# pierotofy/OpenSplat

Hardware: NVIDIA H100
Metric: fwd_bwd_mpixel_per_s (higher is better)
Workload: dtype f32

## Files before the change

opensplat_b200/csrc/raster_bwd.cu:

```cuda
#include "raster_common.cuh"

int gsb_blend_grid(const void *kernel, int num_tiles);

namespace {

__device__ __forceinline__ float rcp_approx(float x) {
    float y;
    asm("rcp.approx.ftz.f32 %0, %1;" : "=f"(y) : "f"(x));
    return y;
}

__device__ __forceinline__ void zero_row(float *grad_rows, int k) {
    float4 *row = reinterpret_cast<float4 *>(grad_rows + (size_t)k * GSB_GRAD_ROW_FLOATS);
    const float4 z = make_float4(0.f, 0.f, 0.f, 0.f);
    row[0] = z; row[1] = z; row[2] = z;
}

constexpr int BWD_MIN_BLOCKS = 6;
template <bool SAT>
__global__ void __launch_bounds__(RK_THREADS, BWD_MIN_BLOCKS)
rasterize_backward_kernel(int img_h, int img_w, int tiles_x, int num_tiles,
                          const int2 *__restrict__ tile_bins, const GsbRecord *__restrict__ records,
                          const float *__restrict__ background, const float *__restrict__ final_Ts,
                          const int *__restrict__ final_idx, const float *__restrict__ v_output,
                          const float *__restrict__ v_output_alpha, float *__restrict__ grad_rows,
                          unsigned *__restrict__ tile_counter, const int *__restrict__ tile_order) {
    __shared__ WarpRing rings[RK_WARPS];
    const int warp = threadIdx.x >> 5, lane = threadIdx.x & 31;
    WarpRing &ring = rings[warp];
    if (lane == 0) {
#pragma unroll
        for (int s = 0; s < RK_STAGES; ++s) mbar_init(&ring.full[s], 1);
        mbar_fence_init();
    }
    __syncwarp();
    const float bg0 = __ldg(background), bg1 = __ldg(background + 1), bg2 = __ldg(background + 2);
    unsigned gchunk = 0;

    while (true) {
        int tile = 0;
        if (lane == 0) tile = (int)atomicAdd(tile_counter, 1u);
        tile = __shfl_sync(0xffffffffu, tile, 0);
        if (tile >= num_tiles) break;
        if (tile_order) tile = __ldg(tile_order + tile);
        const int2 range = tile_bins[tile];
        if (range.y <= range.x) continue;

        const int tx = tile % tiles_x, ty = tile / tiles_x;
        const int X = tx * GSB_TILE + (lane & 15);
        const int Y0 = ty * GSB_TILE + (lane >> 4);
        const float px = (float)X;
        const float tile_x0 = (float)(tx * GSB_TILE), tile_y0 = (float)(ty * GSB_TILE);

        float T[RK_PIX], Bq[RK_PIX];
        const float py0 = (float)Y0;
        float vor[RK_PIX], vog[RK_PIX], vob[RK_PIX];
        int binf[RK_PIX];
        int my_max = -1;
#pragma unroll
        for (int j = 0; j < RK_PIX; ++j) {
            const int Y = Y0 + 2 * j;
            if (X < img_w && Y < img_h) {
                const size_t p = (size_t)Y * img_w + X;
                const float Tf = final_Ts[p];
                T[j] = Tf;
                vor[j] = v_output[3 * p]; vog[j] = v_output[3 * p + 1]; vob[j] = v_output[3 * p + 2];
                binf[j] = final_idx[p];
                if (SAT) {
                    const int f = binf[j];
                    if (f & GSB_SAT_BIT0) vor[j] = 0.f;
                    if (f & (GSB_SAT_BIT0 << 1)) vog[j] = 0.f;
                    if (f & (GSB_SAT_BIT0 << 2)) vob[j] = 0.f;
                    binf[j] = f & ~GSB_SAT_MASK;
                }
                const float voa = v_output_alpha ? v_output_alpha[p] : 0.f;
                Bq[j] = -(Tf * (voa - (bg0 * vor[j] + bg1 * vog[j] + bg2 * vob[j])));
            } else {
                T[j] = 1.f; vor[j] = vog[j] = vob[j] = 0.f; Bq[j] = 0.f;
                binf[j] = -1;
            }
            my_max = max(my_max, binf[j]);
        }
        const int warp_max = __reduce_max_sync(0xffffffffu, my_max);
        const int hi = min(range.y - 1, max(warp_max, range.x - 1));

        for (int idx = hi + 1 + lane; idx < range.y; idx += 32)
            zero_row(grad_rows, __float_as_int(__ldg(&records[idx].q0.w)));
        const int L = hi - range.x + 1;
        if (L <= 0) continue;
        const int nchunks = (L + RK_CHUNK - 1) / RK_CHUNK;

        const unsigned g0 = gchunk;
        auto stage_of = [&](int c) { return (g0 + (unsigned)c) % RK_STAGES; };
        auto parity_of = [&](int c) { return ((g0 + (unsigned)c) / RK_STAGES) & 1u; };
        auto chunk_lo = [&](int c) { return max(range.x, hi + 1 - (c + 1) * RK_CHUNK); };
        auto chunk_cnt = [&](int c) { return (hi + 1 - c * RK_CHUNK) - chunk_lo(c); };
        auto issue = [&](int c) {
            if (lane == 0) {
                const unsigned s = stage_of(c);
                const uint32_t bytes = (uint32_t)chunk_cnt(c) * (uint32_t)sizeof(GsbRecord);
                mbar_arrive_expect_tx(&ring.full[s], bytes);
                tma_load_1d(&ring.rec[s][0], records + chunk_lo(c), bytes, &ring.full[s]);
            }
        };
        const int pro = min(RK_STAGES, nchunks);
        for (int c = 0; c < pro; ++c) issue(c);
        int issued = pro;

        for (int c = 0; c < nchunks; ++c) {
            const unsigned s = stage_of(c);
            mbar_wait(&ring.full[s], parity_of(c));
            const int lo = chunk_lo(c), cnt = chunk_cnt(c);
            unsigned my_mask = 0;
            if (lane < cnt) {
                my_mask = record_slot_mask(ring.rec[s][lane], tile_x0, tile_y0);
                if (my_mask == 0u) zero_row(grad_rows, __float_as_int(ring.rec[s][lane].q0.w));
            }
            unsigned live = __ballot_sync(0xffffffffu, my_mask != 0u);
            while (live) {
                const int t = 31 - __clz(live);
                live &= ~(1u << t);
                const unsigned rm = __shfl_sync(0xffffffffu, my_mask, t);
                const int idx = lo + t;
                const float4 q0 = ring.rec[s][t].q0;
                const float4 q1 = ring.rec[s][t].q1;
                const float4 q2 = ring.rec[s][t].q2;
                const float smax = fmaxf(0.f, fmaf(q0.z, GSB_LN2, GSB_SMAX_BIAS));
                const float dx = q0.x - px;
                const float adx2 = q1.x * dx * dx;
                const float bdx = q1.y * dx;
                const float dy0 = q0.y - py0;
                float s0 = 0.f, s1 = 0.f, s2 = 0.f;
                float a_r = 0.f, a_g = 0.f, a_b = 0.f;
                bool any = false;
                const int jlo = __ffs(rm) - 1, jhi = 31 - __clz(rm);
#define GSB_BWD_SLOT(j)                                                                                   \
    {                                                                                                     \
        const float dy = dy0 - (float)(2 * j);                                                                      \
        const float sigma = fmaf(dy, fmaf(q1.z, dy, bdx), adx2);                                          \
        if (__float_as_uint(sigma) <= __float_as_uint(smax)) {                    \
            const float au = ex2_approx(fmaf(sigma, -GSB_LOG2E, q0.z));           \
            const float alpha = fminf(0.99f, au);                                                         \
            if (idx <= binf[j] && alpha >= (1.f / 255.f)) {                                               \
                any = true;                                                                               \
                const float ra = rcp_approx(1.f - alpha);                                                 \
                T[j] *= ra;                                                                               \
                const float fac = alpha * T[j];                                                           \
                a_r = fmaf(fac, vor[j], a_r);                                                             \
                a_g = fmaf(fac, vog[j], a_g);                                                             \
                a_b = fmaf(fac, vob[j], a_b);                                                             \
                const float d = fmaf(q2.z, vob[j], fmaf(q2.y, vog[j], q2.x * vor[j]));   \
                const float v_alpha = fmaf(d, T[j], -(ra * Bq[j]));                                       \
                Bq[j] = fmaf(d, fac, Bq[j]);                                                              \
                 \
                const float w = au * v_alpha;                                                             \
                const float wdy = w * dy;                                                                 \
                s0 += w;                                                                                  \
                s1 += wdy;                                                                                \
                s2 = fmaf(wdy, dy, s2);                                                                   \
            }                                                                                             \
        }                                                                                                 \
        if (jhi == j) break;                                                                              \
    }
                switch (jlo) {
                    case 0: GSB_BWD_SLOT(0)
                    case 1: GSB_BWD_SLOT(1)
                    case 2: GSB_BWD_SLOT(2)
                    case 3: GSB_BWD_SLOT(3)
                    case 4: GSB_BWD_SLOT(4)
                    case 5: GSB_BWD_SLOT(5)
                    case 6: GSB_BWD_SLOT(6)
                    default: GSB_BWD_SLOT(7)
                }
#undef GSB_BWD_SLOT
                const int k = __float_as_int(q0.w);
                float *row = grad_rows + (size_t)k * GSB_GRAD_ROW_FLOATS;
                if (!__any_sync(0xffffffffu, any)) {
                    if (lane < 9) row[lane] = 0.f;
                    continue;
                }
                const float sx = dx * s0;
                float v0 = s0, v1 = sx, v2 = s1, v3 = dx * sx, v4 = dx * s1, v5 = s2, v6 = a_r, v7 = a_g;
                float v8 = a_b;
                {
                    const bool up = lane & 16;
                    const float t0 = up ? v0 : v4, t1 = up ? v1 : v5, t2 = up ? v2 : v6, t3 = up ? v3 : v7;
                    const float k0 = up ? v4 : v0, k1 = up ? v5 : v1, k2 = up ? v6 : v2, k3 = up ? v7 : v3;
                    v0 = k0 + __shfl_xor_sync(0xffffffffu, t0, 16);
                    v1 = k1 + __shfl_xor_sync(0xffffffffu, t1, 16);
                    v2 = k2 + __shfl_xor_sync(0xffffffffu, t2, 16);
                    v3 = k3 + __shfl_xor_sync(0xffffffffu, t3, 16);
                }
                {
                    const bool up = lane & 8;
                    const float t0 = up ? v0 : v2, t1 = up ? v1 : v3;
                    const float k0 = up ? v2 : v0, k1 = up ? v3 : v1;
                    v0 = k0 + __shfl_xor_sync(0xffffffffu, t0, 8);
                    v1 = k1 + __shfl_xor_sync(0xffffffffu, t1, 8);
                }
                {
                    const bool up = lane & 4;
                    const float t0 = up ? v0 : v1;
                    const float k0 = up ? v1 : v0;
                    v0 = k0 + __shfl_xor_sync(0xffffffffu, t0, 4);
                }
                v0 += __shfl_xor_sync(0xffffffffu, v0, 2);
                v0 += __shfl_xor_sync(0xffffffffu, v0, 1);
#pragma unroll
                for (int o = 16; o > 0; o >>= 1) v8 += __shfl_xor_sync(0xffffffffu, v8, o);
                const bool w8 = (lane == 1);
                if (((lane & 3) == 0) || w8) row[w8 ? 8 : (lane >> 2)] = w8 ? v8 : v0;
            }
            __syncwarp();
            if (issued < nchunks) { issue(issued); ++issued; }
        }
        gchunk = g0 + (unsigned)issued;
        __syncwarp();
    }
}

__global__ void __launch_bounds__(256)
reduce_grad_rows_kernel(int n, const int *__restrict__ cum_tiles_hit, const float *__restrict__ grad_rows,
                        const float *__restrict__ conics, const float *__restrict__ opacities,
                        float2 *__restrict__ v_xy, float *__restrict__ v_conic,
                        float *__restrict__ v_colors, float *__restrict__ v_opacity) {
    const int g = blockIdx.x * blockDim.x + threadIdx.x;
    if (g >= n) return;
    const int k0 = g ? cum_tiles_hit[g - 1] : 0, k1 = cum_tiles_hit[g];
    float a[9] = {0.f, 0.f, 0.f, 0.f, 0.f, 0.f, 0.f, 0.f, 0.f};
    for (int k = k0; k < k1; ++k) {
        const float4 *row = reinterpret_cast<const float4 *>(grad_rows + (size_t)k * GSB_GRAD_ROW_FLOATS);
        const float4 r0 = row[0], r1 = row[1];
        const float r8 = reinterpret_cast<const float *>(row)[8];
        a[0] += r0.x; a[1] += r0.y; a[2] += r0.z; a[3] += r0.w;
        a[4] += r1.x; a[5] += r1.y; a[6] += r1.z; a[7] += r1.w;
        a[8] += r8;
    }
    const float S0 = a[0], Sx = a[1], Sy = a[2], Sxx = a[3], Sxy = a[4], Syy = a[5];
    const float ca = conics[3 * g], cb = conics[3 * g + 1], cc = conics[3 * g + 2];
    const float op = opacities[g];
    v_xy[g] = make_float2(-(ca * Sx + cb * Sy), -(cb * Sx + cc * Sy));
    v_conic[3 * g] = -0.5f * Sxx; v_conic[3 * g + 1] = -0.5f * Sxy; v_conic[3 * g + 2] = -0.5f * Syy;
    v_colors[3 * g] = a[6]; v_colors[3 * g + 1] = a[7]; v_colors[3 * g + 2] = a[8];
    v_opacity[g] = (op > 0.f) ? S0 / op : 0.f;
}

}

extern "C" size_t gsb_raster_grad_rows_bytes(int m) {
    return gsb_align_up((size_t)(m > 0 ? m : 0) * GSB_GRAD_ROW_FLOATS * 4 + 256, 256);
}

extern "C" int gsb_rasterize_backward(int img_h, int img_w, int tiles_x, int tiles_y, int n, int m,
                                      const int32_t *tile_bins, const int32_t *tile_order, const float *conics,
                                      const float *opacities, void *records, const int32_t *cum_tiles_hit,
                                      const float *background, const float *final_Ts, const int32_t *final_idx,
                                      const float *v_output, const float *v_output_alpha, void *grad_rows,
                                      float *v_xy, float *v_conic, float *v_colors, float *v_opacity, unsigned flags,
                                      gsb_stream_t stream) {
    GSB_CHECK_ARG(img_h > 0 && img_w > 0 && n >= 0 && m >= 0);
    GSB_CHECK_ARG((flags & ~(unsigned)GSB_RASTER_CLAMP_MAX_ONE) == 0);
    const bool sat = (flags & GSB_RASTER_CLAMP_MAX_ONE) != 0;
    GSB_CHECK_ARG(tiles_x == gsb_div_up(img_w, GSB_TILE) && tiles_y == gsb_div_up(img_h, GSB_TILE));
    if (n == 0) return 0;
    GSB_CHECK_ARG(tile_bins && conics && opacities && cum_tiles_hit && background && final_Ts && final_idx &&
                  v_output && v_xy && v_conic && v_colors && v_opacity);
    GSB_CHECK_ARG(((uintptr_t)v_xy % 8) == 0);
    cudaStream_t s = (cudaStream_t)stream;
    if (m > 0) {
        GSB_CHECK_ARG(records && grad_rows && ((uintptr_t)records % 16) == 0 && ((uintptr_t)grad_rows % 16) == 0);
        unsigned *counters = reinterpret_cast<unsigned *>(
            reinterpret_cast<char *>(records) + gsb_raster_records_bytes(m) - 256);
        GSB_CUDA(cudaMemsetAsync(counters, 0, 256, s));
        const int num_tiles = tiles_x * tiles_y;
#define GSB_BWD_LAUNCH(S)                                                                                       \
    rasterize_backward_kernel<S><<<gsb_blend_grid((const void *)rasterize_backward_kernel<S>, num_tiles),        \
                                   RK_THREADS, 0, s>>>(                                                         \
        img_h, img_w, tiles_x, num_tiles, reinterpret_cast<const int2 *>(tile_bins),                            \
        reinterpret_cast<const GsbRecord *>(records), background, final_Ts, final_idx, v_output, v_output_alpha, \
        reinterpret_cast<float *>(grad_rows), counters, tile_order)
        if (sat) GSB_BWD_LAUNCH(true); else GSB_BWD_LAUNCH(false);
#undef GSB_BWD_LAUNCH
    }
    reduce_grad_rows_kernel<<<gsb_div_up(n, 256), 256, 0, s>>>(
        n, cum_tiles_hit, reinterpret_cast<const float *>(grad_rows), conics, opacities,
        reinterpret_cast<float2 *>(v_xy), v_conic, v_colors, v_opacity);
    GSB_LAUNCH_CHECK();
    return 0;
}
```

opensplat_b200/csrc/raster_common.cuh:

```cuda
#pragma once
#include "gsb_common.cuh"

struct __align__(16) GsbRecord {
    float4 q0, q1, q2;
};
static_assert(sizeof(GsbRecord) == 48, "record must be 48 bytes");

constexpr int RK_WARPS = 4;
constexpr int RK_THREADS = RK_WARPS * 32;
constexpr int RK_PIX = 8;
constexpr int RK_CHUNK = 32;
constexpr int RK_STAGES = 4;

constexpr float GSB_LN2 = 0.6931471805599453f;
constexpr float GSB_LOG2E = 1.4426950408889634f;
constexpr float GSB_SMAX_BIAS = 5.541263545158426f + 1e-3f;

constexpr int GSB_GRAD_ROW_FLOATS = 12;

constexpr int GSB_SAT_BIT0 = 1 << 28;
constexpr int GSB_SAT_MASK = 7 << 28;

struct __align__(128) WarpRing {
    GsbRecord rec[RK_STAGES][RK_CHUNK];
    uint64_t full[RK_STAGES];
};

#ifdef __CUDACC__
__device__ __forceinline__ GsbRecord make_record(float2 xy, float a, float b, float c, float opac, float r,
                                                 float g, float bl, int k) {
    const float lo = (opac > 0.f) ? log2f(opac) : -INFINITY;
    const float smax = fmaxf(0.f, fmaf(lo, GSB_LN2, GSB_SMAX_BIAS));
    const float det = a * c - b * b;
    float hx = INFINITY, hy = INFINITY;
    if (det > 0.f && a > 0.f && c > 0.f) {
        const float s2 = 2.f * smax / det;
        hx = sqrtf(s2 * c) * 1.001f + 0.01f;
        hy = sqrtf(s2 * a) * 1.001f + 0.01f;
    }
    GsbRecord rec;
    rec.q0 = make_float4(xy.x, xy.y, lo, __int_as_float(k));
    rec.q1 = make_float4(0.5f * a, b, 0.5f * c, hx);
    rec.q2 = make_float4(r, g, bl, hy);
    return rec;
}

__device__ __forceinline__ unsigned extent_slot_mask(float cx, float cy, float hx, float hy, float tile_x0,
                                                     float tile_y0) {
    const float gx = cx - tile_x0, gy = cy - tile_y0;
    const float xlo = fmaxf(ceilf(gx - hx), 0.f), xhi = fminf(floorf(gx + hx), 15.f);
    const float ylo = fmaxf(ceilf(gy - hy), 0.f), yhi = fminf(floorf(gy + hy), 15.f);
    if (!(xlo <= xhi) || !(ylo <= yhi)) return 0u;
    const int jlo = (int)ylo >> 1, jhi = (int)yhi >> 1;
    return ((2u << jhi) - 1u) & ~((1u << jlo) - 1u);
}

__device__ __forceinline__ unsigned record_slot_mask(const GsbRecord &r, float tile_x0, float tile_y0) {
    return extent_slot_mask(r.q0.x, r.q0.y, r.q1.w, r.q2.w, tile_x0, tile_y0);
}
#endif
```

opensplat_b200/csrc/raster_fwd.cu:

```cuda
#include "raster_common.cuh"

namespace {

__global__ void __launch_bounds__(256)
pack_records_kernel(int m, const int *__restrict__ gaussian_ids_sorted,
                    const int *__restrict__ sorted_index, const float2 *__restrict__ xys,
                    const float *__restrict__ conics, const float *__restrict__ colors,
                    const float *__restrict__ opacities, GsbRecord *__restrict__ records) {
    const int i = blockIdx.x * blockDim.x + threadIdx.x;
    if (i >= m) return;
    const int g = gaussian_ids_sorted[i];
    const int k = sorted_index ? sorted_index[i] : i;
    const GsbRecord r = make_record(__ldg(xys + g), __ldg(conics + 3 * g), __ldg(conics + 3 * g + 1),
                                    __ldg(conics + 3 * g + 2), __ldg(opacities + g), __ldg(colors + 3 * g),
                                    __ldg(colors + 3 * g + 1), __ldg(colors + 3 * g + 2), k);
    float4 *dst = reinterpret_cast<float4 *>(records + i);
    stg_stream4(dst, r.q0);
    stg_stream4(dst + 1, r.q1);
    stg_stream4(dst + 2, r.q2);
}

constexpr int FWD_MIN_BLOCKS = 8;
template <bool COUNT, bool SAT>
__global__ void __launch_bounds__(RK_THREADS, FWD_MIN_BLOCKS)
rasterize_forward_kernel(int img_h, int img_w, int tiles_x, int num_tiles,
                         const int2 *__restrict__ tile_bins, const GsbRecord *__restrict__ records,
                         const float *__restrict__ background, float *__restrict__ out_img,
                         float *__restrict__ final_Ts, int *__restrict__ final_idx,
                         unsigned *__restrict__ tile_counter, const int *__restrict__ bin_stats,
                         unsigned long long *__restrict__ pair_counts, const int *__restrict__ tile_order) {
    if (bin_stats && bin_stats[2]) return;
    __shared__ WarpRing rings[RK_WARPS];
    const int warp = threadIdx.x >> 5, lane = threadIdx.x & 31;
    WarpRing &ring = rings[warp];
    if (lane == 0) {
#pragma unroll
        for (int s = 0; s < RK_STAGES; ++s) mbar_init(&ring.full[s], 1);
        mbar_fence_init();
    }
    __syncwarp();
    const float bg0 = __ldg(background), bg1 = __ldg(background + 1), bg2 = __ldg(background + 2);
    unsigned gchunk = 0;
    unsigned long long n_rec = 0, n_slot = 0, n_eval = 0, n_blend = 0;

    while (true) {
        int tile = 0;
        if (lane == 0) tile = (int)atomicAdd(tile_counter, 1u);
        tile = __shfl_sync(0xffffffffu, tile, 0);
        if (tile >= num_tiles) break;
        if (tile_order) tile = __ldg(tile_order + tile);

        const int tx = tile % tiles_x, ty = tile / tiles_x;
        const int X = tx * GSB_TILE + (lane & 15);
        const int Y0 = ty * GSB_TILE + (lane >> 4);
        const float px = (float)X;
        const float tile_x0 = (float)(tx * GSB_TILE), tile_y0 = (float)(ty * GSB_TILE);
        const int2 range = tile_bins[tile];
        const int L = range.y - range.x;
        const int nchunks = (L + RK_CHUNK - 1) / RK_CHUNK;

        float T[RK_PIX], cr[RK_PIX], cg[RK_PIX], cb[RK_PIX];
        const float py0 = (float)Y0;
        int last[RK_PIX];
        unsigned done = 0;
#pragma unroll
        for (int j = 0; j < RK_PIX; ++j) {
            T[j] = 1.f; cr[j] = cg[j] = cb[j] = 0.f; last[j] = 0;
            if (X >= img_w || Y0 + 2 * j >= img_h) { done |= 1u << j; T[j] = -1.f; }
        }

        const unsigned g0 = gchunk;
        auto stage_of = [&](int c) { return (g0 + (unsigned)c) % RK_STAGES; };
        auto parity_of = [&](int c) { return ((g0 + (unsigned)c) / RK_STAGES) & 1u; };
        auto issue = [&](int c) {
            if (lane == 0) {
                const int cnt = min(RK_CHUNK, L - c * RK_CHUNK);
                const uint32_t bytes = (uint32_t)cnt * (uint32_t)sizeof(GsbRecord);
                const unsigned s = stage_of(c);
                mbar_arrive_expect_tx(&ring.full[s], bytes);
                tma_load_1d(&ring.rec[s][0], records + range.x + c * RK_CHUNK, bytes, &ring.full[s]);
            }
        };
        const int pro = min(RK_STAGES, nchunks);
        for (int c = 0; c < pro; ++c) issue(c);
        int issued = pro;

        int c = 0;
        for (; c < nchunks; ++c) {
            const unsigned s = stage_of(c);
            mbar_wait(&ring.full[s], parity_of(c));
            const int cnt = min(RK_CHUNK, L - c * RK_CHUNK);
            const int idx0 = range.x + c * RK_CHUNK;
            unsigned my_mask = 0;
            if (lane < cnt) my_mask = record_slot_mask(ring.rec[s][lane], tile_x0, tile_y0);
            unsigned live = __ballot_sync(0xffffffffu, my_mask != 0u);
            if (COUNT && lane == 0) n_rec += __popc(live);
            while (live) {
                const int t = __ffs(live) - 1;
                live &= live - 1;
                const unsigned rm = __shfl_sync(0xffffffffu, my_mask, t);
                const float4 q0 = ring.rec[s][t].q0;
                const float4 q1 = ring.rec[s][t].q1;
                const float4 q2 = ring.rec[s][t].q2;
                const float smax = fmaxf(0.f, fmaf(q0.z, GSB_LN2, GSB_SMAX_BIAS));
                const float dx = q0.x - px;
                const float adx2 = q1.x * dx * dx;
                const float bdx = q1.y * dx;
                const float dy0 = q0.y - py0;
                const int idx = idx0 + t;
                const int jhi = 31 - __clz(rm);
#define GSB_FWD_SLOT(j)                                                                                   \
    {                                                                                                     \
        const float dy = dy0 - (float)(2 * j);                                                                      \
                                      \
        const float sigma = fmaf(dy, fmaf(q1.z, dy, bdx), adx2);                                          \
        if (COUNT && lane == 0) ++n_slot;                                                                 \
        if (__float_as_uint(sigma) <= __float_as_uint(smax)) {            \
                     \
            const float alpha = fminf(0.999f, ex2_approx(fmaf(sigma, -GSB_LOG2E, q0.z)));                 \
            if (COUNT) ++n_eval;                                                                          \
            if (alpha >= (1.f / 255.f)) {                                                                 \
                const float next_T = T[j] * (1.f - alpha);                                                \
                if (next_T <= 1e-4f) {                                     \
                    if (T[j] > 0.f) { T[j] = -T[j]; done |= 1u << j; }                                    \
                } else {                                                                                  \
                    const float vis = alpha * T[j];                                                       \
                    cr[j] = fmaf(q2.x, vis, cr[j]);                                                       \
                    cg[j] = fmaf(q2.y, vis, cg[j]);                                                       \
                    cb[j] = fmaf(q2.z, vis, cb[j]);                                                       \
                    T[j] = next_T;                                                                        \
                    last[j] = idx;                                                                        \
                    if (COUNT) ++n_blend;                                                                 \
                }                                                                                         \
            }                                                                                             \
        }                                                                                                 \
        if (jhi == j) break;                                                                              \
    }
                do {
                    if (rm & 1u) GSB_FWD_SLOT(0)
                    if (rm & 2u) GSB_FWD_SLOT(1)
                    if (rm & 4u) GSB_FWD_SLOT(2)
                    if (rm & 8u) GSB_FWD_SLOT(3)
                    if (rm & 16u) GSB_FWD_SLOT(4)
                    if (rm & 32u) GSB_FWD_SLOT(5)
                    if (rm & 64u) GSB_FWD_SLOT(6)
                    if (rm & 128u) GSB_FWD_SLOT(7)
                } while (0);
#undef GSB_FWD_SLOT
            }
            if (__all_sync(0xffffffffu, done == 0xffu)) { ++c; break; }
            __syncwarp();
            if (issued < nchunks) { issue(issued); ++issued; }
        }
        for (; c < issued; ++c) mbar_wait(&ring.full[stage_of(c)], parity_of(c));
        gchunk = g0 + (unsigned)issued;
        __syncwarp();

#pragma unroll
        for (int j = 0; j < RK_PIX; ++j) {
            const int Y = Y0 + 2 * j;
            if (X < img_w && Y < img_h) {
                const size_t p = (size_t)Y * img_w + X;
                const float Tf = fabsf(T[j]);
                final_Ts[p] = Tf;
                float o0 = cr[j] + Tf * bg0, o1 = cg[j] + Tf * bg1, o2 = cb[j] + Tf * bg2;
                int fi = last[j];
                if (SAT) {
                    if (!(o0 <= 1.f)) { fi |= GSB_SAT_BIT0; o0 = o0 > 1.f ? 1.f : o0; }
                    if (!(o1 <= 1.f)) { fi |= GSB_SAT_BIT0 << 1; o1 = o1 > 1.f ? 1.f : o1; }
                    if (!(o2 <= 1.f)) { fi |= GSB_SAT_BIT0 << 2; o2 = o2 > 1.f ? 1.f : o2; }
                }
                final_idx[p] = fi;
                out_img[3 * p] = o0;
                out_img[3 * p + 1] = o1;
                out_img[3 * p + 2] = o2;
            }
        }
    }
    if (COUNT) {
        n_eval = __reduce_add_sync(0xffffffffu, (unsigned)n_eval);
        n_blend = __reduce_add_sync(0xffffffffu, (unsigned)n_blend);
        if (lane == 0) {
            atomicAdd(pair_counts + 0, n_rec);
            atomicAdd(pair_counts + 1, n_slot);
            atomicAdd(pair_counts + 2, n_eval);
            atomicAdd(pair_counts + 3, n_blend);
        }
    }
}


}

int gsb_sm_count();
int gsb_blend_grid(const void *kernel, int num_tiles);

extern "C" size_t gsb_raster_records_bytes(int m) {
    return gsb_align_up((size_t)(m > 0 ? m : 0) * sizeof(GsbRecord), 256) + 256;
}

extern "C" int gsb_pack_records(int m, const int32_t *gaussian_ids_sorted, const int32_t *sorted_index,
                                const float *xys, const float *conics, const float *colors, const float *opacities,
                                void *records, gsb_stream_t stream) {
    GSB_CHECK_ARG(m >= 0);
    if (m == 0) return 0;
    GSB_CHECK_ARG(records && gaussian_ids_sorted && xys && conics && colors && opacities);
    GSB_CHECK_ARG(((uintptr_t)records % 16) == 0 && ((uintptr_t)xys % 8) == 0);
    pack_records_kernel<<<gsb_div_up(m, 256), 256, 0, (cudaStream_t)stream>>>(
        m, gaussian_ids_sorted, sorted_index, reinterpret_cast<const float2 *>(xys), conics, colors, opacities,
        reinterpret_cast<GsbRecord *>(records));
    GSB_LAUNCH_CHECK();
    return 0;
}

static int blend_setup(int img_h, int img_w, int tiles_x, int tiles_y, int m, const int32_t *tile_bins,
                       const float *background, void *records, float *out_img, float *final_Ts, int32_t *final_idx,
                       cudaStream_t s, unsigned **counters) {
    GSB_CHECK_ARG(img_h > 0 && img_w > 0 && m >= 0);
    GSB_CHECK_ARG(tiles_x == gsb_div_up(img_w, GSB_TILE) && tiles_y == gsb_div_up(img_h, GSB_TILE));
    GSB_CHECK_ARG(tile_bins && background && out_img && final_Ts && final_idx && records);
    GSB_CHECK_ARG(((uintptr_t)records % 16) == 0);
    *counters = reinterpret_cast<unsigned *>(reinterpret_cast<char *>(records) + gsb_raster_records_bytes(m) - 256);
    GSB_CUDA(cudaMemsetAsync(*counters, 0, 256, s));
    return 0;
}

extern "C" int gsb_rasterize_forward_packed(int img_h, int img_w, int tiles_x, int tiles_y, int m,
                                            const int32_t *tile_bins, const int32_t *tile_order,
                                            const int32_t *bin_stats, const float *background, void *records,
                                            float *out_img, float *final_Ts, int32_t *final_idx, unsigned flags,
                                            gsb_stream_t stream) {
    GSB_CHECK_ARG((flags & ~(unsigned)GSB_RASTER_CLAMP_MAX_ONE) == 0);
    const bool sat = (flags & GSB_RASTER_CLAMP_MAX_ONE) != 0;
    GSB_CHECK_ARG(!sat || m < GSB_SAT_BIT0);
    cudaStream_t s = (cudaStream_t)stream;
    unsigned *counters = nullptr;
    const int rc = blend_setup(img_h, img_w, tiles_x, tiles_y, m, tile_bins, background, records, out_img, final_Ts,
                               final_idx, s, &counters);
    if (rc) return rc;
    const int num_tiles = tiles_x * tiles_y;
#define GSB_FWD_LAUNCH(S)                                                                                        \
    rasterize_forward_kernel<false, S><<<gsb_blend_grid((const void *)rasterize_forward_kernel<false, S>, num_tiles), \
                                         RK_THREADS, 0, s>>>(                                                    \
        img_h, img_w, tiles_x, num_tiles, reinterpret_cast<const int2 *>(tile_bins),                             \
        reinterpret_cast<const GsbRecord *>(records), background, out_img, final_Ts, final_idx, counters,        \
        bin_stats, nullptr, tile_order)
    if (sat) GSB_FWD_LAUNCH(true); else GSB_FWD_LAUNCH(false);
#undef GSB_FWD_LAUNCH
    GSB_LAUNCH_CHECK();
    return 0;
}

extern "C" int gsb_rasterize_forward_count(int img_h, int img_w, int tiles_x, int tiles_y, int m,
                                           const int32_t *tile_bins, const float *background, void *records,
                                           float *out_img, float *final_Ts, int32_t *final_idx,
                                           unsigned long long *pair_counts, gsb_stream_t stream) {
    GSB_CHECK_ARG(pair_counts);
    cudaStream_t s = (cudaStream_t)stream;
    unsigned *counters = nullptr;
    const int rc = blend_setup(img_h, img_w, tiles_x, tiles_y, m, tile_bins, background, records, out_img, final_Ts,
                               final_idx, s, &counters);
    if (rc) return rc;
    const int num_tiles = tiles_x * tiles_y;
    const int grid = gsb_blend_grid((const void *)rasterize_forward_kernel<true, false>, num_tiles);
    rasterize_forward_kernel<true, false><<<grid, RK_THREADS, 0, s>>>(
        img_h, img_w, tiles_x, num_tiles, reinterpret_cast<const int2 *>(tile_bins),
        reinterpret_cast<const GsbRecord *>(records), background, out_img, final_Ts, final_idx, counters, nullptr,
        pair_counts, nullptr);
    GSB_LAUNCH_CHECK();
    return 0;
}

int gsb_sm_count() {
    static thread_local int cached_dev = -1, cached = 0;
    int dev = 0;
    cudaGetDevice(&dev);
    if (dev != cached_dev) {
        cudaDeviceGetAttribute(&cached, cudaDevAttrMultiProcessorCount, dev);
        if (cached <= 0) cached = 132;
        cached_dev = dev;
    }
    return cached;
}

int gsb_blend_grid(const void *kernel, int num_tiles) {
    struct Entry { const void *kernel; int dev; int per_sm; };
    static thread_local Entry cache[8] = {};
    int dev = 0;
    cudaGetDevice(&dev);
    int per_sm = 0;
    for (const Entry &e : cache)
        if (e.kernel == kernel && e.dev == dev) per_sm = e.per_sm;
    if (per_sm == 0) {
        if (cudaOccupancyMaxActiveBlocksPerMultiprocessor(&per_sm, kernel, RK_THREADS, 0) != cudaSuccess || per_sm < 1)
            per_sm = 1;
        for (Entry &e : cache)
            if (e.kernel == nullptr || e.kernel == kernel) { e = Entry{kernel, dev, per_sm}; break; }
    }
    const int full = gsb_sm_count() * per_sm;
    const int need = gsb_div_up(num_tiles, RK_WARPS);
    return need < full ? need : full;
}
```

Before: 1087.

## Remap forward warp pixels to 8x4 quads with 2D slot culling masks

The forward rasterizer now has each lane cover two columns (X0 and X0+8) across four row groups instead of one column across eight rows. A new slot mask culls Gaussians by both x-half and y-quad, and the x-dependent conic terms are computed once per column and shared across rows. The backward kernel keeps the old row-pair mask under a new name. The goal is tighter per-slot culling so fewer sigma evaluations run; in exchange the forward kernel carries more registers, which is why min blocks drops from 8 to 7.

```diff
diff --git a/opensplat_b200/csrc/raster_bwd.cu b/opensplat_b200/csrc/raster_bwd.cu
--- a/opensplat_b200/csrc/raster_bwd.cu
+++ b/opensplat_b200/csrc/raster_bwd.cu
@@ -113,7 +113,8 @@
             const int lo = chunk_lo(c), cnt = chunk_cnt(c);
             unsigned my_mask = 0;
             if (lane < cnt) {
-                my_mask = record_slot_mask(ring.rec[s][lane], tile_x0, tile_y0);
+                const GsbRecord &r = ring.rec[s][lane];
+                my_mask = extent_row_pair_mask(r.q0.x, r.q0.y, r.q1.w, r.q2.w, tile_x0, tile_y0);
                 if (my_mask == 0u) zero_row(grad_rows, __float_as_int(ring.rec[s][lane].q0.w));
             }
             unsigned live = __ballot_sync(0xffffffffu, my_mask != 0u);
diff --git a/opensplat_b200/csrc/raster_common.cuh b/opensplat_b200/csrc/raster_common.cuh
--- a/opensplat_b200/csrc/raster_common.cuh
+++ b/opensplat_b200/csrc/raster_common.cuh
@@ -45,17 +45,28 @@
     return rec;
 }
 
+__device__ __forceinline__ bool extent_box(float cx, float cy, float hx, float hy, float tile_x0, float tile_y0,
+                                           int &xlo, int &xhi, int &ylo, int &yhi) {
+    const float gx = cx - tile_x0, gy = cy - tile_y0;
+    const float fxlo = fmaxf(ceilf(gx - hx), 0.f), fxhi = fminf(floorf(gx + hx), 15.f);
+    const float fylo = fmaxf(ceilf(gy - hy), 0.f), fyhi = fminf(floorf(gy + hy), 15.f);
+    if (!(fxlo <= fxhi) || !(fylo <= fyhi)) return false;
+    xlo = (int)fxlo; xhi = (int)fxhi; ylo = (int)fylo; yhi = (int)fyhi;
+    return true;
+}
+
 __device__ __forceinline__ unsigned extent_slot_mask(float cx, float cy, float hx, float hy, float tile_x0,
                                                      float tile_y0) {
-    const float gx = cx - tile_x0, gy = cy - tile_y0;
-    const float xlo = fmaxf(ceilf(gx - hx), 0.f), xhi = fminf(floorf(gx + hx), 15.f);
-    const float ylo = fmaxf(ceilf(gy - hy), 0.f), yhi = fminf(floorf(gy + hy), 15.f);
-    if (!(xlo <= xhi) || !(ylo <= yhi)) return 0u;
-    const int jlo = (int)ylo >> 1, jhi = (int)yhi >> 1;
-    return ((2u << jhi) - 1u) & ~((1u << jlo) - 1u);
+    int xlo, xhi, ylo, yhi;
+    if (!extent_box(cx, cy, hx, hy, tile_x0, tile_y0, xlo, xhi, ylo, yhi)) return 0u;
+    const unsigned quads = 0x55u & ((4u << (2 * (yhi >> 2))) - 1u) & ~((1u << (2 * (ylo >> 2))) - 1u);
+    return (quads << (xlo >> 3)) | (quads << (xhi >> 3));
 }
 
-__device__ __forceinline__ unsigned record_slot_mask(const GsbRecord &r, float tile_x0, float tile_y0) {
-    return extent_slot_mask(r.q0.x, r.q0.y, r.q1.w, r.q2.w, tile_x0, tile_y0);
+__device__ __forceinline__ unsigned extent_row_pair_mask(float cx, float cy, float hx, float hy, float tile_x0,
+                                                         float tile_y0) {
+    int xlo, xhi, ylo, yhi;
+    if (!extent_box(cx, cy, hx, hy, tile_x0, tile_y0, xlo, xhi, ylo, yhi)) return 0u;
+    return ((2u << (yhi >> 1)) - 1u) & ~((1u << (ylo >> 1)) - 1u);
 }
 #endif
diff --git a/opensplat_b200/csrc/raster_fwd.cu b/opensplat_b200/csrc/raster_fwd.cu
--- a/opensplat_b200/csrc/raster_fwd.cu
+++ b/opensplat_b200/csrc/raster_fwd.cu
@@ -20,7 +20,7 @@
     stg_stream4(dst + 2, r.q2);
 }
 
-constexpr int FWD_MIN_BLOCKS = 8;
+constexpr int FWD_MIN_BLOCKS = 7;
 template <bool COUNT, bool SAT>
 __global__ void __launch_bounds__(RK_THREADS, FWD_MIN_BLOCKS)
 rasterize_forward_kernel(int img_h, int img_w, int tiles_x, int num_tiles,
@@ -51,22 +51,22 @@
         if (tile_order) tile = __ldg(tile_order + tile);
 
         const int tx = tile % tiles_x, ty = tile / tiles_x;
-        const int X = tx * GSB_TILE + (lane & 15);
-        const int Y0 = ty * GSB_TILE + (lane >> 4);
-        const float px = (float)X;
+        const int X0 = tx * GSB_TILE + (lane & 7);
+        const int Y0 = ty * GSB_TILE + (lane >> 3);
+        const float px0 = (float)X0, px1 = (float)(X0 + 8);
         const float tile_x0 = (float)(tx * GSB_TILE), tile_y0 = (float)(ty * GSB_TILE);
         const int2 range = tile_bins[tile];
         const int L = range.y - range.x;
         const int nchunks = (L + RK_CHUNK - 1) / RK_CHUNK;
 
         float T[RK_PIX], cr[RK_PIX], cg[RK_PIX], cb[RK_PIX];
-        const float py0 = (float)Y0;
+        const float py0 = (float)(ty * GSB_TILE + (lane >> 3 & 1)), row_off = (float)(lane >> 3 & 2);
         int last[RK_PIX];
         unsigned done = 0;
 #pragma unroll
         for (int j = 0; j < RK_PIX; ++j) {
             T[j] = 1.f; cr[j] = cg[j] = cb[j] = 0.f; last[j] = 0;
-            if (X >= img_w || Y0 + 2 * j >= img_h) { done |= 1u << j; T[j] = -1.f; }
+            if (X0 + 8 * (j & 1) >= img_w || Y0 + 4 * (j >> 1) >= img_h) { done |= 1u << j; T[j] = -1.f; }
         }
 
         const unsigned g0 = gchunk;
@@ -92,7 +92,10 @@
             const int cnt = min(RK_CHUNK, L - c * RK_CHUNK);
             const int idx0 = range.x + c * RK_CHUNK;
             unsigned my_mask = 0;
-            if (lane < cnt) my_mask = record_slot_mask(ring.rec[s][lane], tile_x0, tile_y0);
+            if (lane < cnt) {
+                const GsbRecord &r = ring.rec[s][lane];
+                my_mask = extent_slot_mask(r.q0.x, r.q0.y, r.q1.w, r.q2.w, tile_x0, tile_y0);
+            }
             unsigned live = __ballot_sync(0xffffffffu, my_mask != 0u);
             if (COUNT && lane == 0) n_rec += __popc(live);
             while (live) {
@@ -103,17 +106,12 @@
                 const float4 q1 = ring.rec[s][t].q1;
                 const float4 q2 = ring.rec[s][t].q2;
                 const float smax = fmaxf(0.f, fmaf(q0.z, GSB_LN2, GSB_SMAX_BIAS));
-                const float dx = q0.x - px;
-                const float adx2 = q1.x * dx * dx;
-                const float bdx = q1.y * dx;
+                const float dx0 = q0.x - px0, dx1 = q0.x - px1;
+                const float adx2_0 = q1.x * dx0 * dx0, adx2_1 = q1.x * dx1 * dx1;
+                const float bdx0 = q1.y * dx0, bdx1 = q1.y * dx1;
                 const float dy0 = q0.y - py0;
                 const int idx = idx0 + t;
-                const int jhi = 31 - __clz(rm);
-#define GSB_FWD_SLOT(j)                                                                                   \
-    {                                                                                                     \
-        const float dy = dy0 - (float)(2 * j);                                                                      \
-                                      \
-        const float sigma = fmaf(dy, fmaf(q1.z, dy, bdx), adx2);                                          \
+#define GSB_FWD_BODY(j)                                                                                   \
         if (COUNT && lane == 0) ++n_slot;                                                                 \
         if (__float_as_uint(sigma) <= __float_as_uint(smax)) {            \
                      \
@@ -133,20 +131,21 @@
                     if (COUNT) ++n_blend;                                                                 \
                 }                                                                                         \
             }                                                                                             \
-        }                                                                                                 \
-        if (jhi == j) break;                                                                              \
-    }
-                do {
-                    if (rm & 1u) GSB_FWD_SLOT(0)
-                    if (rm & 2u) GSB_FWD_SLOT(1)
-                    if (rm & 4u) GSB_FWD_SLOT(2)
-                    if (rm & 8u) GSB_FWD_SLOT(3)
-                    if (rm & 16u) GSB_FWD_SLOT(4)
-                    if (rm & 32u) GSB_FWD_SLOT(5)
-                    if (rm & 64u) GSB_FWD_SLOT(6)
-                    if (rm & 128u) GSB_FWD_SLOT(7)
-                } while (0);
+        }
+
+#define GSB_FWD_SLOT(j, bdx, adx2) { const float sigma = fmaf(dy, fmaf(q1.z, dy, bdx), adx2); GSB_FWD_BODY(j) }
+#define GSB_S(q)                                                                                          \
+    if (rm & (3u << (2 * (q)))) {                                                                         \
+        const float dy = dy0 - (row_off + (float)(4 * (q)));                    \
+                                      \
+        if (rm & (1u << (2 * (q)))) GSB_FWD_SLOT(2 * (q), bdx0, adx2_0)                                   \
+        if (rm & (2u << (2 * (q)))) GSB_FWD_SLOT(2 * (q) + 1, bdx1, adx2_1)                               \
+        if (rm < (4u << (2 * (q)))) break;                                      \
+    }
+                do { GSB_S(0) GSB_S(1) GSB_S(2) GSB_S(3) } while (0);
+#undef GSB_S
 #undef GSB_FWD_SLOT
+#undef GSB_FWD_BODY
             }
             if (__all_sync(0xffffffffu, done == 0xffu)) { ++c; break; }
             __syncwarp();
@@ -158,7 +157,7 @@
 
 #pragma unroll
         for (int j = 0; j < RK_PIX; ++j) {
-            const int Y = Y0 + 2 * j;
+            const int X = X0 + 8 * (j & 1), Y = Y0 + 4 * (j >> 1);
             if (X < img_w && Y < img_h) {
                 const size_t p = (size_t)Y * img_w + X;
                 const float Tf = fabsf(T[j]);
```

Result: faster. 1100, median of 6 (+1.2%).
